# facebookresearch/fast3r

Measured on NVIDIA H100. Metric: views_per_sec, higher is better.
Workload: dtype bf16

## Files before the change

### fast3r_b200/csrc/gemm.cu

```cuda
#include "common.cuh"
#include "f3r_kernels.h"

namespace f3r {

constexpr int BLOCK_M = 128;
constexpr int BLOCK_K = 64;
constexpr int GEMM_THREADS = 384;
constexpr int XCH_STRIDE = 68;

template <int BLOCK_N>
struct GemmCfg {
  static constexpr int kStages = (BLOCK_N == 256) ? 3 : 4;
  static constexpr int kABytes = BLOCK_M * BLOCK_K * 2;
  static constexpr int kBBytes = BLOCK_N * BLOCK_K * 2;
  static constexpr int kStageBytes = kABytes + kBBytes;
  static constexpr int kXchBytes = 64 * XCH_STRIDE * 4;
  static constexpr int kSmemBytes =
      kStages * kStageBytes + 1024  + 1024  + 8 * 4096  + 2 * kXchBytes;
};

struct ResChunk {
  uint4 r0[8];
  uint2 r1[8];
};

__device__ __forceinline__ size_t out_offset(const GemmArgs& p, int m, int col0, int img, int py, int px) {
  if (p.epi == EPI_CONVT) {
    const int ij = col0 / p.ct_cout, o0 = col0 % p.ct_cout, k = p.ct_k;
    const int oy = py * k + ij / k, ox = px * k + ij % k;
    return ((static_cast<size_t>(img) * p.H * k + oy) * (p.W * k) + ox) * p.ct_cout + o0;
  }
  return static_cast<size_t>(m) * p.ldo + col0;
}

__device__ __forceinline__ void prefetch_res(const GemmArgs& p, ResChunk& rc, size_t off_row, bool ok_row, int lane) {
  if (p.res0 == nullptr && p.res1 == nullptr) return;
  const unsigned okmask = __ballot_sync(0xffffffffu, ok_row);
#pragma unroll
  for (int i = 0; i < 8; ++i) {
    const int rr = 4 * i + (lane >> 3);
    const size_t off = __shfl_sync(0xffffffffu, off_row, rr) + (lane & 7) * 4;
    if (!((okmask >> rr) & 1)) continue;
    if (p.res0 != nullptr) {
      if (p.res0_f32) rc.r0[i] = *reinterpret_cast<const uint4*>(static_cast<const float*>(p.res0) + off);
      else {
        const uint2 t = *reinterpret_cast<const uint2*>(static_cast<const __nv_bfloat16*>(p.res0) + off);
        rc.r0[i].x = t.x; rc.r0[i].y = t.y;
      }
    }
    if (p.res1 != nullptr) rc.r1[i] = *reinterpret_cast<const uint2*>(static_cast<const __nv_bfloat16*>(p.res1) + off);
  }
}

__device__ __forceinline__ void gelu_fast(float& x) {
  const float z = __fmul_rn(fabsf(x), 0.70710678118654752440f);
  const float u = fmaf(z, 0.3275911f, 1.0f);
  float t;
  asm("rcp.approx.ftz.f32 %0, %1;" : "=f"(t) : "f"(u));
  float q = fmaf(t, 1.061405429f, -1.453152027f);
  q = fmaf(q, t, 1.421413741f);
  q = fmaf(q, t, -0.284496736f);
  q = fmaf(q, t, 0.254829592f);
  q = __fmul_rn(q, t);
  const float a = __fmul_rn(__fmul_rn(z, z), -1.4426950408889634f);
  float e;
  asm("ex2.approx.ftz.f32 %0, %1;" : "=f"(e) : "f"(a));
  const float r = copysignf(fmaf(q, -e, 1.0f), x);
  const float h = __fmul_rn(x, 0.5f);
  x = fmaf(h, r, h);
}
__device__ __forceinline__ bool epilogue_rows(const GemmArgs& p, float (&v)[32], int m, int col0, bool row_ok,
                                              float (&fin)[4], bool add_bias, const float* w4s) {
  if (p.bias != nullptr && add_bias) {
    const float4* b4 = reinterpret_cast<const float4*>(p.bias + (p.epi == EPI_CONVT ? (col0 % p.ct_cout) : col0));
#pragma unroll
    for (int i = 0; i < 8; ++i) {
      float4 b = __ldg(b4 + i);
      v[4 * i + 0] += b.x; v[4 * i + 1] += b.y; v[4 * i + 2] += b.z; v[4 * i + 3] += b.w;
    }
  }
  if (p.epi == EPI_ROPE && col0 < p.rope_cols && row_ok) {
    const int t = m % p.tok_per_img;
    const int pos = ((col0 >> 5) & 1) ? (t % p.grid_w) : (t / p.grid_w);
    const float4* c4 = reinterpret_cast<const float4*>(p.rope_cos + pos * 16);
    const float4* s4 = reinterpret_cast<const float4*>(p.rope_sin + pos * 16);
#pragma unroll
    for (int i = 0; i < 4; ++i) {
      float4 c = __ldg(c4 + i), s = __ldg(s4 + i);
      float cc[4] = {c.x, c.y, c.z, c.w}, ss[4] = {s.x, s.y, s.z, s.w};
#pragma unroll
      for (int e = 0; e < 4; ++e) {
        const int j = 4 * i + e;
        const float a = v[j], b = v[j + 16];
        v[j] = a * cc[e] - b * ss[e];
        v[j + 16] = b * cc[e] + a * ss[e];
      }
    }
  }
  if (p.epi == EPI_IDXEMB && row_ok) {
    const int id = __ldg(p.emb_ids + (p.tok_per_img > 0 ? m / p.tok_per_img : m));
    const float4* e4 = reinterpret_cast<const float4*>(p.emb_table + static_cast<size_t>(id) * p.N + col0);
#pragma unroll
    for (int i = 0; i < 8; ++i) {
      float4 e = __ldg(e4 + i);
      v[4 * i + 0] += e.x; v[4 * i + 1] += e.y; v[4 * i + 2] += e.z; v[4 * i + 3] += e.w;
    }
  }
  if (p.epi == EPI_FINAL) {
    if (row_ok) {
#pragma unroll
      for (int o = 0; o < 4; ++o) {
        const float4* w = reinterpret_cast<const float4*>(w4s + o * p.N + col0);
        float acc = fin[o];
#pragma unroll
        for (int i = 0; i < 8; ++i) {
          const float4 ww = w[i];
          acc = fmaf(fmaxf(v[4 * i + 0], 0.f), ww.x, acc);
          acc = fmaf(fmaxf(v[4 * i + 1], 0.f), ww.y, acc);
          acc = fmaf(fmaxf(v[4 * i + 2], 0.f), ww.z, acc);
          acc = fmaf(fmaxf(v[4 * i + 3], 0.f), ww.w, acc);
        }
        fin[o] = acc;
      }
    }
    return false;
  }
  return true;
}

__device__ __forceinline__ void epilogue_store(const GemmArgs& p, const float (&v)[32], const ResChunk& rc, uint8_t* stage,
                                               int lane, int m, int col0, size_t off_row, bool ok_row) {
#pragma unroll
  for (int j = 0; j < 8; ++j)
    *reinterpret_cast<float4*>(stage + lane * 128 + ((j ^ (lane & 7)) << 4)) =
        make_float4(v[4 * j], v[4 * j + 1], v[4 * j + 2], v[4 * j + 3]);
  __syncwarp();
  const unsigned okmask = __ballot_sync(0xffffffffu, ok_row);
  const int cj = lane & 7;
  const bool to_b = p.split_col > 0 && col0 >= p.split_col;
#pragma unroll
  for (int i = 0; i < 8; ++i) {
    const int rr = 4 * i + (lane >> 3);
    const size_t off = __shfl_sync(0xffffffffu, off_row, rr) + cj * 4;
    const int mrow = __shfl_sync(0xffffffffu, m, rr);
    if (!((okmask >> rr) & 1)) continue;
    const float4 a = *reinterpret_cast<const float4*>(stage + rr * 128 + ((cj ^ (rr & 7)) << 4));
    float x0 = a.x, x1 = a.y, x2 = a.z, x3 = a.w;
    if (p.res0 != nullptr) {
      if (p.res0_f32) {
        x0 += __uint_as_float(rc.r0[i].x); x1 += __uint_as_float(rc.r0[i].y);
        x2 += __uint_as_float(rc.r0[i].z); x3 += __uint_as_float(rc.r0[i].w);
      } else {
        x0 += bf16_lo(rc.r0[i].x); x1 += bf16_hi(rc.r0[i].x); x2 += bf16_lo(rc.r0[i].y); x3 += bf16_hi(rc.r0[i].y);
      }
    }
    if (p.res1 != nullptr) {
      x0 += bf16_lo(rc.r1[i].x); x1 += bf16_hi(rc.r1[i].x); x2 += bf16_lo(rc.r1[i].y); x3 += bf16_hi(rc.r1[i].y);
    }
    if (p.out1 != nullptr) {
      uint2 o;
      o.x = pack_bf16(fmaxf(x0, 0.f), fmaxf(x1, 0.f));
      o.y = pack_bf16(fmaxf(x2, 0.f), fmaxf(x3, 0.f));
      *reinterpret_cast<uint2*>(static_cast<__nv_bfloat16*>(p.out1) + off) = o;
    }
    if (p.out0 == nullptr) continue;
    if (p.act == ACT_RELU) {
      x0 = fmaxf(x0, 0.f); x1 = fmaxf(x1, 0.f); x2 = fmaxf(x2, 0.f); x3 = fmaxf(x3, 0.f);
    } else if (p.act == ACT_GELU) {
      gelu_fast(x0); gelu_fast(x1); gelu_fast(x2); gelu_fast(x3);
    }
    void* base = p.out0;
    size_t o = off;
    if (to_b) {
      base = p.out0b;
      o = static_cast<size_t>(mrow) * p.ldo_b + (col0 - p.split_col) + cj * 4;
    }
    if (p.out0_f32) {
      *reinterpret_cast<float4*>(static_cast<float*>(base) + o) = make_float4(x0, x1, x2, x3);
    } else {
      uint2 q;
      q.x = pack_bf16(x0, x1);
      q.y = pack_bf16(x2, x3);
      *reinterpret_cast<uint2*>(static_cast<__nv_bfloat16*>(base) + o) = q;
    }
  }
  __syncwarp();
}

__device__ __forceinline__ void epilogue_tma(const GemmArgs& p, float (&v)[32], uint8_t* stage, int lane,
                                             const CUtensorMap* map, bool reduce, int c_col, int c_x, int c_y, int c_img) {
  if (p.act == ACT_RELU) {
#pragma unroll
    for (int i = 0; i < 32; ++i) v[i] = fmaxf(v[i], 0.f);
  } else if (p.act == ACT_GELU) {
#pragma unroll
    for (int i = 0; i < 32; ++i) gelu_fast(v[i]);
  }
  if (lane == 0) tma_store_wait_read();
  __syncwarp();
  if (p.out0_f32) {
#pragma unroll
    for (int j = 0; j < 8; ++j)
      *reinterpret_cast<float4*>(stage + lane * 128 + ((j ^ (lane & 7)) << 4)) =
          make_float4(v[4 * j], v[4 * j + 1], v[4 * j + 2], v[4 * j + 3]);
  } else {
#pragma unroll
    for (int j = 0; j < 4; ++j) {
      uint4 q;
      q.x = pack_bf16(v[8 * j + 0], v[8 * j + 1]);
      q.y = pack_bf16(v[8 * j + 2], v[8 * j + 3]);
      q.z = pack_bf16(v[8 * j + 4], v[8 * j + 5]);
      q.w = pack_bf16(v[8 * j + 6], v[8 * j + 7]);
      *reinterpret_cast<uint4*>(stage + lane * 64 + ((j ^ ((lane >> 1) & 3)) << 4)) = q;
    }
  }
  fence_proxy_async_smem();
  __syncwarp();
  if (lane == 0) {
    if (reduce) tma_reduce_add_4d(map, stage, c_col, c_x, c_y, c_img);
    else tma_store_4d(map, stage, c_col, c_x, c_y, c_img);
    tma_store_commit();
  }
}

template <int BLOCK_N>
__global__ void __launch_bounds__(GEMM_THREADS, 1)
gemm_kernel(const __grid_constant__ CUtensorMap tmap_a, const __grid_constant__ CUtensorMap tmap_b,
            const __grid_constant__ CUtensorMap tmap_o0, const __grid_constant__ CUtensorMap tmap_o0b,
            const __grid_constant__ GemmArgs p) {
  using Cfg = GemmCfg<BLOCK_N>;
  extern __shared__ uint8_t smem_raw[];
  uint8_t* smem = reinterpret_cast<uint8_t*>((reinterpret_cast<uintptr_t>(smem_raw) + 1023) & ~uintptr_t(1023));
  uint8_t* smem_a = smem;
  uint8_t* smem_b = smem + Cfg::kStages * Cfg::kABytes;
  uint64_t* bars = reinterpret_cast<uint64_t*>(smem + Cfg::kStages * Cfg::kStageBytes);
  uint64_t* full_bar = bars;
  uint64_t* empty_bar = bars + Cfg::kStages;
  uint8_t* stage_base = smem + Cfg::kStages * Cfg::kStageBytes + 1024;
  float* fin_smem = reinterpret_cast<float*>(stage_base);
  float* w4_smem = reinterpret_cast<float*>(stage_base + 4096);
  float* xch_base = reinterpret_cast<float*>(stage_base + 8 * 4096);

  const int warp = threadIdx.x >> 5;
  const int lane = threadIdx.x & 31;

  if (threadIdx.x == 0) {
    tma_prefetch_desc(&tmap_a);
    tma_prefetch_desc(&tmap_b);
    for (int s = 0; s < Cfg::kStages; ++s) { mbar_init(&full_bar[s], 1); mbar_init(&empty_bar[s], 2); }
    fence_barrier_init();
  }
  if (p.epi == EPI_FINAL)
    for (int i = threadIdx.x; i < 4 * p.N; i += GEMM_THREADS) w4_smem[i] = __ldg(p.w4 + i);
  __syncthreads();
  pdl_wait();
  pdl_launch_dependents();

  const int num_out_tiles = p.num_m_tiles * p.num_n_tiles;
  const int num_tiles = num_out_tiles * p.k_split;
  const int k_chunks = (p.K + BLOCK_K - 1) / BLOCK_K;
  const int k_iters = p.taps * k_chunks;

  if (warp < 4) {
    asm volatile("setmaxnreg.dec.sync.aligned.u32 40;");
    if (warp == 0 && lane == 0) {
      int stage = 0; uint32_t phase = 0;
      for (int item = blockIdx.x; item < num_tiles; item += gridDim.x) {
        const int tile = item % num_out_tiles, ks = item / num_out_tiles;
        const int it0 = ks * k_iters / p.k_split, it1 = (ks + 1) * k_iters / p.k_split;
        const int mt = tile / p.num_n_tiles, nt = tile % p.num_n_tiles;
        const int tx = mt % p.tiles_x, ty = (mt / p.tiles_x) % p.tiles_y, img = mt / (p.tiles_x * p.tiles_y);
        const int x0 = tx * p.bw, y0 = ty * p.bh, n0 = nt * BLOCK_N;
        for (int it = it0; it < it1; ++it) {
          const int tap = it / k_chunks, kc = it % k_chunks;
          int dy = 0, dx = 0;
          if (p.taps == 9) { dy = tap / 3 - 1; dx = tap % 3 - 1; }
          mbar_wait_relaxed(&empty_bar[stage], phase ^ 1);
          mbar_arrive_expect_tx(&full_bar[stage], Cfg::kStageBytes);
          tma_load_4d(smem_a + stage * Cfg::kABytes, &tmap_a, &full_bar[stage], kc * BLOCK_K, x0 + dx, y0 + dy, img);
          tma_load_3d(smem_b + stage * Cfg::kBBytes, &tmap_b, &full_bar[stage], kc * BLOCK_K, tap, n0);
          if (++stage == Cfg::kStages) { stage = 0; phase ^= 1; }
        }
      }
    }
  } else {
    asm volatile("setmaxnreg.inc.sync.aligned.u32 232;");
    const int cg = (warp - 4) >> 2;
    const int wg_warp = warp & 3;
    const int wg_tid = threadIdx.x & 127;
    const int half = wg_warp >> 1;
    const int r_loc = (wg_warp & 1) * 32 + lane;
    const int r = cg * 64 + r_loc;
    float* xch = xch_base + cg * 64 * XCH_STRIDE;
    uint8_t* stage_buf = stage_base + (warp - 4) * 4096;
    const int bar_id = 1 + cg;
    constexpr int kAcc = BLOCK_N / 2;
    int stage = 0; uint32_t phase = 0;
    for (int item = blockIdx.x; item < num_tiles; item += gridDim.x) {
      const int tile = item % num_out_tiles, ks = item / num_out_tiles;
      const int it0 = ks * k_iters / p.k_split, it1 = (ks + 1) * k_iters / p.k_split;
      const bool add_bias = ks == 0;
      float acc[kAcc];
#pragma unroll
      for (int i = 0; i < kAcc; ++i) acc[i] = 0.f;
      int prev = -1;
      for (int it = it0; it < it1; ++it) {
        mbar_wait(&full_bar[stage], phase);
        const uint64_t a_desc = make_smem_desc_sw128(smem_u32(smem_a + stage * Cfg::kABytes + cg * 64 * 128));
        const uint64_t b_desc = make_smem_desc_sw128(smem_u32(smem_b + stage * Cfg::kBBytes));
        fence_regs(acc);
        wgmma_fence();
#pragma unroll
        for (int k = 0; k < BLOCK_K / 16; ++k) {
          if constexpr (BLOCK_N == 256) wgmma_ss_n256<0>(acc, a_desc + 2 * k, b_desc + 2 * k, 1u);
          else wgmma_ss_n128<0>(acc, a_desc + 2 * k, b_desc + 2 * k, 1u);
        }
        wgmma_commit();
        wgmma_wait<1>();
        fence_regs(acc);
        if (prev >= 0 && wg_tid == 0) mbar_arrive(&empty_bar[prev]);
        prev = stage;
        if (++stage == Cfg::kStages) { stage = 0; phase ^= 1; }
      }
      wgmma_wait<0>();
      fence_regs(acc);
      if (prev >= 0 && wg_tid == 0) mbar_arrive(&empty_bar[prev]);

      const int mt = tile / p.num_n_tiles, nt = tile % p.num_n_tiles;
      const int tx = mt % p.tiles_x, ty = (mt / p.tiles_x) % p.tiles_y, img = mt / (p.tiles_x * p.tiles_y);
      const int px = tx * p.bw + r % p.bw, py = ty * p.bh + r / p.bw;
      const bool row_ok = (px < p.W) && (py < p.H) && (mt < p.num_m_tiles);
      const int m = (img * p.H + py) * p.W + px;
      const int n_valid = min(BLOCK_N / 32, (p.N - nt * BLOCK_N + 31) / 32);
      float fin[4] = {0.f, 0.f, 0.f, 0.f};
#pragma unroll
      for (int cp = 0; cp < BLOCK_N / 64; ++cp) {
        asm volatile("bar.sync %0, 128;" ::"r"(bar_id) : "memory");
        {
          const int fr = wg_warp * 16 + (lane >> 2), fc = 2 * (lane & 3);
#pragma unroll
          for (int j = 0; j < 8; ++j) {
            const int jj = cp * 8 + j;
            *reinterpret_cast<float2*>(xch + fr * XCH_STRIDE + 8 * j + fc) = make_float2(acc[4 * jj], acc[4 * jj + 1]);
            *reinterpret_cast<float2*>(xch + (fr + 8) * XCH_STRIDE + 8 * j + fc) =
                make_float2(acc[4 * jj + 2], acc[4 * jj + 3]);
          }
        }
        asm volatile("bar.sync %0, 128;" ::"r"(bar_id) : "memory");
        const int c = 2 * cp + half;
        if (c >= n_valid) continue;
        const int col0 = nt * BLOCK_N + c * 32;
        float v[32];
#pragma unroll
        for (int i = 0; i < 8; ++i) {
          const float4 t = *reinterpret_cast<const float4*>(xch + r_loc * XCH_STRIDE + half * 32 + 4 * i);
          v[4 * i] = t.x; v[4 * i + 1] = t.y; v[4 * i + 2] = t.z; v[4 * i + 3] = t.w;
        }
        if (epilogue_rows(p, v, m, col0, row_ok, fin, add_bias, w4_smem) && !(p.debug & 1)) {
          if (p.tma_epi) {
            const bool to_b = p.split_col > 0 && col0 >= p.split_col;
            const int r0 = cg * 64 + (wg_warp & 1) * 32;
            epilogue_tma(p, v, stage_buf, lane, to_b ? &tmap_o0b : &tmap_o0, p.tma_epi == 2,
                         to_b ? col0 - p.split_col : col0, tx * p.bw + (r0 & (p.bw - 1)), ty * p.bh + (r0 >> p.bw_log2),
                         mt < p.num_m_tiles ? img : p.NB);
          } else {
            const size_t off = out_offset(p, m, col0, img, py, px);
            ResChunk rc;
            prefetch_res(p, rc, off, row_ok, lane);
            epilogue_store(p, v, rc, stage_buf, lane, m, col0, off, row_ok);
          }
        }
      }
      if (p.epi == EPI_FINAL) {
        float* slot = fin_smem + r * 4;
        if (half == 1) { slot[0] = fin[0]; slot[1] = fin[1]; slot[2] = fin[2]; slot[3] = fin[3]; }
        asm volatile("bar.sync %0, 128;" ::"r"(bar_id) : "memory");
        if (half == 0 && row_ok) {
          const float x = fin[0] + slot[0] + __ldg(p.b4 + 0), y = fin[1] + slot[1] + __ldg(p.b4 + 1);
          const float z = fin[2] + slot[2] + __ldg(p.b4 + 2), c = fin[3] + slot[3] + __ldg(p.b4 + 3);
          const float d = sqrtf(x * x + y * y + z * z);
          const float sc = expm1f(d) / fmaxf(d, 1e-8f);
          float* pt = p.pts + static_cast<size_t>(m) * 3;
          pt[0] = x * sc; pt[1] = y * sc; pt[2] = z * sc;
          p.conf[m] = 1.f + expf(c);
        }
      }
    }
    if (p.tma_epi && lane == 0) tma_store_wait_all();
  }
}

template <int BLOCK_N>
static cudaError_t launch_gemm_t(const CUtensorMap& ta, const CUtensorMap& tb, const CUtensorMap& to0,
                                 const CUtensorMap& to0b, const GemmArgs& a, int num_sms, cudaStream_t stream) {
  const int items = a.num_m_tiles * a.num_n_tiles * a.k_split;
  return launch(gemm_kernel<BLOCK_N>, items < num_sms ? items : num_sms, GEMM_THREADS, GemmCfg<BLOCK_N>::kSmemBytes,
                stream, true, ta, tb, to0, to0b, a);
}

cudaError_t launch_gemm(int block_n, const CUtensorMap& ta, const CUtensorMap& tb, const CUtensorMap& to0,
                        const CUtensorMap& to0b, const GemmArgs& a, int num_sms, cudaStream_t stream) {
  if (block_n == 256) return launch_gemm_t<256>(ta, tb, to0, to0b, a, num_sms, stream);
  return launch_gemm_t<128>(ta, tb, to0, to0b, a, num_sms, stream);
}

}
```

Baseline: 149.1.

## Run GEMM epilogue directly on MMA fragments instead of shared-memory transpose

The epilogue now applies bias, RoPE and index embeddings directly on the wgmma accumulator fragment layout. This removes the per-chunk shared-memory exchange and the two 128-thread barriers that converted fragments to row-per-thread form. Warps are paired to share a double-buffered TMA staging area synchronized with 64-thread named barriers. Freeing the exchange buffer lets BLOCK_N=256 use four pipeline stages instead of three, while the FINAL epilogue keeps the old exchange path for BLOCK_N=128. In exchange the indexing and synchronization become more complex.

```diff
diff --git a/fast3r_b200/csrc/gemm.cu b/fast3r_b200/csrc/gemm.cu
--- a/fast3r_b200/csrc/gemm.cu
+++ b/fast3r_b200/csrc/gemm.cu
@@ -10,18 +10,19 @@
 
 template <int BLOCK_N>
 struct GemmCfg {
-  static constexpr int kStages = (BLOCK_N == 256) ? 3 : 4;
+  static constexpr int kStages = 4;
   static constexpr int kABytes = BLOCK_M * BLOCK_K * 2;
   static constexpr int kBBytes = BLOCK_N * BLOCK_K * 2;
   static constexpr int kStageBytes = kABytes + kBBytes;
-  static constexpr int kXchBytes = 64 * XCH_STRIDE * 4;
+  static constexpr int kXchBytes = (BLOCK_N == 128) ? 2 * 64 * XCH_STRIDE * 4 : 0;
   static constexpr int kSmemBytes =
-      kStages * kStageBytes + 1024  + 1024  + 8 * 4096  + 2 * kXchBytes;
+      kStages * kStageBytes + 1024  + 1024  + 8 * 4096  + kXchBytes;
 };
+static_assert(GemmCfg<256>::kSmemBytes <= 227 * 1024 && GemmCfg<128>::kSmemBytes <= 227 * 1024, "shared memory per CTA");
 
 struct ResChunk {
-  uint4 r0[8];
-  uint2 r1[8];
+  uint4 r0[4];
+  uint2 r1[4];
 };
 
 __device__ __forceinline__ size_t out_offset(const GemmArgs& p, int m, int col0, int img, int py, int px) {
@@ -33,14 +34,21 @@
   return static_cast<size_t>(m) * p.ldo + col0;
 }
 
-__device__ __forceinline__ void prefetch_res(const GemmArgs& p, ResChunk& rc, size_t off_row, bool ok_row, int lane) {
+struct FragRows {
+  int m[2];
+  int px[2], py[2];
+  bool ok[2];
+};
+
+__device__ __forceinline__ void prefetch_res(const GemmArgs& p, ResChunk& rc, const size_t (&off_row)[2], const FragRows& rows,
+                                             int lane) {
   if (p.res0 == nullptr && p.res1 == nullptr) return;
-  const unsigned okmask = __ballot_sync(0xffffffffu, ok_row);
-#pragma unroll
-  for (int i = 0; i < 8; ++i) {
-    const int rr = 4 * i + (lane >> 3);
-    const size_t off = __shfl_sync(0xffffffffu, off_row, rr) + (lane & 7) * 4;
-    if (!((okmask >> rr) & 1)) continue;
+  const unsigned okmask[2] = {__ballot_sync(0xffffffffu, rows.ok[0]), __ballot_sync(0xffffffffu, rows.ok[1])};
+#pragma unroll
+  for (int i = 0; i < 4; ++i) {
+    const int src = 4 * ((4 * i + (lane >> 3)) & 7);
+    const size_t off = __shfl_sync(0xffffffffu, off_row[i >> 1], src) + (lane & 7) * 4;
+    if (!((okmask[i >> 1] >> src) & 1)) continue;
     if (p.res0 != nullptr) {
       if (p.res0_f32) rc.r0[i] = *reinterpret_cast<const uint4*>(static_cast<const float*>(p.res0) + off);
       else {
@@ -69,81 +77,111 @@
   const float h = __fmul_rn(x, 0.5f);
   x = fmaf(h, r, h);
 }
-__device__ __forceinline__ bool epilogue_rows(const GemmArgs& p, float (&v)[32], int m, int col0, bool row_ok,
-                                              float (&fin)[4], bool add_bias, const float* w4s) {
+template <int kAcc>
+__device__ __forceinline__ void epilogue_frag(const GemmArgs& p, float (&acc)[kAcc], int c, int col0, const FragRows& rows,
+                                              int lane, bool add_bias) {
+  const int t2 = 2 * (lane & 3);
   if (p.bias != nullptr && add_bias) {
-    const float4* b4 = reinterpret_cast<const float4*>(p.bias + (p.epi == EPI_CONVT ? (col0 % p.ct_cout) : col0));
+    const float2* b2 = reinterpret_cast<const float2*>(p.bias + (p.epi == EPI_CONVT ? (col0 % p.ct_cout) : col0) + t2);
+#pragma unroll
+    for (int jl = 0; jl < 4; ++jl) {
+      const float2 b = __ldg(b2 + 4 * jl);
+#pragma unroll
+      for (int h = 0; h < 2; ++h) { acc[16 * c + 4 * jl + 2 * h] += b.x; acc[16 * c + 4 * jl + 2 * h + 1] += b.y; }
+    }
+  }
+  if (p.epi == EPI_ROPE && col0 < p.rope_cols) {
+#pragma unroll
+    for (int h = 0; h < 2; ++h) {
+      if (!rows.ok[h]) continue;
+      const int t = rows.m[h] % p.tok_per_img;
+      const int pos = ((col0 >> 5) & 1) ? (t % p.grid_w) : (t / p.grid_w);
+      const float2* c2 = reinterpret_cast<const float2*>(p.rope_cos + pos * 16 + t2);
+      const float2* s2 = reinterpret_cast<const float2*>(p.rope_sin + pos * 16 + t2);
+#pragma unroll
+      for (int jl = 0; jl < 2; ++jl) {
+        const float2 cs = __ldg(c2 + 4 * jl), sn = __ldg(s2 + 4 * jl);
+#pragma unroll
+        for (int e = 0; e < 2; ++e) {
+          float& x = acc[16 * c + 4 * jl + 2 * h + e];
+          float& y = acc[16 * c + 4 * (jl + 2) + 2 * h + e];
+          const float a = x, b = y, cc = e ? cs.y : cs.x, ss = e ? sn.y : sn.x;
+          x = fmaf(a, cc, -__fmul_rn(b, ss));
+          y = fmaf(a, ss, __fmul_rn(b, cc));
+        }
+      }
+    }
+  }
+  if (p.epi == EPI_IDXEMB) {
+#pragma unroll
+    for (int h = 0; h < 2; ++h) {
+      if (!rows.ok[h]) continue;
+      const int m = rows.m[h];
+      const int id = __ldg(p.emb_ids + (p.tok_per_img > 0 ? m / p.tok_per_img : m));
+      const float2* e2 = reinterpret_cast<const float2*>(p.emb_table + static_cast<size_t>(id) * p.N + col0 + t2);
+#pragma unroll
+      for (int jl = 0; jl < 4; ++jl) {
+        const float2 e = __ldg(e2 + 4 * jl);
+        acc[16 * c + 4 * jl + 2 * h] += e.x; acc[16 * c + 4 * jl + 2 * h + 1] += e.y;
+      }
+    }
+  }
+}
+
+__device__ __forceinline__ void final_rows(const GemmArgs& p, float (&v)[32], int col0, bool row_ok, float (&fin)[4],
+                                           const float* w4s) {
+  if (p.bias != nullptr) {
+    const float4* b4 = reinterpret_cast<const float4*>(p.bias + col0);
 #pragma unroll
     for (int i = 0; i < 8; ++i) {
       float4 b = __ldg(b4 + i);
       v[4 * i + 0] += b.x; v[4 * i + 1] += b.y; v[4 * i + 2] += b.z; v[4 * i + 3] += b.w;
     }
   }
-  if (p.epi == EPI_ROPE && col0 < p.rope_cols && row_ok) {
-    const int t = m % p.tok_per_img;
-    const int pos = ((col0 >> 5) & 1) ? (t % p.grid_w) : (t / p.grid_w);
-    const float4* c4 = reinterpret_cast<const float4*>(p.rope_cos + pos * 16);
-    const float4* s4 = reinterpret_cast<const float4*>(p.rope_sin + pos * 16);
-#pragma unroll
-    for (int i = 0; i < 4; ++i) {
-      float4 c = __ldg(c4 + i), s = __ldg(s4 + i);
-      float cc[4] = {c.x, c.y, c.z, c.w}, ss[4] = {s.x, s.y, s.z, s.w};
-#pragma unroll
-      for (int e = 0; e < 4; ++e) {
-        const int j = 4 * i + e;
-        const float a = v[j], b = v[j + 16];
-        v[j] = a * cc[e] - b * ss[e];
-        v[j + 16] = b * cc[e] + a * ss[e];
-      }
-    }
-  }
-  if (p.epi == EPI_IDXEMB && row_ok) {
-    const int id = __ldg(p.emb_ids + (p.tok_per_img > 0 ? m / p.tok_per_img : m));
-    const float4* e4 = reinterpret_cast<const float4*>(p.emb_table + static_cast<size_t>(id) * p.N + col0);
+  if (!row_ok) return;
+#pragma unroll
+  for (int o = 0; o < 4; ++o) {
+    const float4* w = reinterpret_cast<const float4*>(w4s + o * p.N + col0);
+    float acc = fin[o];
 #pragma unroll
     for (int i = 0; i < 8; ++i) {
-      float4 e = __ldg(e4 + i);
-      v[4 * i + 0] += e.x; v[4 * i + 1] += e.y; v[4 * i + 2] += e.z; v[4 * i + 3] += e.w;
-    }
-  }
-  if (p.epi == EPI_FINAL) {
-    if (row_ok) {
-#pragma unroll
-      for (int o = 0; o < 4; ++o) {
-        const float4* w = reinterpret_cast<const float4*>(w4s + o * p.N + col0);
-        float acc = fin[o];
-#pragma unroll
-        for (int i = 0; i < 8; ++i) {
-          const float4 ww = w[i];
-          acc = fmaf(fmaxf(v[4 * i + 0], 0.f), ww.x, acc);
-          acc = fmaf(fmaxf(v[4 * i + 1], 0.f), ww.y, acc);
-          acc = fmaf(fmaxf(v[4 * i + 2], 0.f), ww.z, acc);
-          acc = fmaf(fmaxf(v[4 * i + 3], 0.f), ww.w, acc);
-        }
-        fin[o] = acc;
-      }
-    }
-    return false;
-  }
-  return true;
-}
-
-__device__ __forceinline__ void epilogue_store(const GemmArgs& p, const float (&v)[32], const ResChunk& rc, uint8_t* stage,
-                                               int lane, int m, int col0, size_t off_row, bool ok_row) {
-#pragma unroll
-  for (int j = 0; j < 8; ++j)
-    *reinterpret_cast<float4*>(stage + lane * 128 + ((j ^ (lane & 7)) << 4)) =
-        make_float4(v[4 * j], v[4 * j + 1], v[4 * j + 2], v[4 * j + 3]);
+      const float4 ww = w[i];
+      acc = fmaf(fmaxf(v[4 * i + 0], 0.f), ww.x, acc);
+      acc = fmaf(fmaxf(v[4 * i + 1], 0.f), ww.y, acc);
+      acc = fmaf(fmaxf(v[4 * i + 2], 0.f), ww.z, acc);
+      acc = fmaf(fmaxf(v[4 * i + 3], 0.f), ww.w, acc);
+    }
+    fin[o] = acc;
+  }
+}
+
+template <int kAcc>
+__device__ __forceinline__ void stage_frag_f32(const float (&acc)[kAcc], int c, uint8_t* stage, int row0, int lane) {
+  const int q = lane >> 2, t = lane & 3;
+#pragma unroll
+  for (int jl = 0; jl < 4; ++jl)
+#pragma unroll
+    for (int h = 0; h < 2; ++h)
+      *reinterpret_cast<float2*>(stage + (row0 + 8 * h) * 128 + (((2 * jl + (t >> 1)) ^ q) << 4) + (t & 1) * 8) =
+          make_float2(acc[16 * c + 4 * jl + 2 * h], acc[16 * c + 4 * jl + 2 * h + 1]);
+}
+
+template <int kAcc>
+__device__ __forceinline__ void epilogue_store(const GemmArgs& p, const float (&acc)[kAcc], int c, const ResChunk& rc,
+                                               uint8_t* stage, int lane, const FragRows& rows, int col0,
+                                               const size_t (&off_row)[2]) {
+  stage_frag_f32(acc, c, stage, lane >> 2, lane);
   __syncwarp();
-  const unsigned okmask = __ballot_sync(0xffffffffu, ok_row);
+  const unsigned okmask[2] = {__ballot_sync(0xffffffffu, rows.ok[0]), __ballot_sync(0xffffffffu, rows.ok[1])};
   const int cj = lane & 7;
   const bool to_b = p.split_col > 0 && col0 >= p.split_col;
 #pragma unroll
-  for (int i = 0; i < 8; ++i) {
+  for (int i = 0; i < 4; ++i) {
     const int rr = 4 * i + (lane >> 3);
-    const size_t off = __shfl_sync(0xffffffffu, off_row, rr) + cj * 4;
-    const int mrow = __shfl_sync(0xffffffffu, m, rr);
-    if (!((okmask >> rr) & 1)) continue;
+    const int src = 4 * (rr & 7);
+    const size_t off = __shfl_sync(0xffffffffu, off_row[i >> 1], src) + cj * 4;
+    const int mrow = __shfl_sync(0xffffffffu, rows.m[i >> 1], src);
+    if (!((okmask[i >> 1] >> src) & 1)) continue;
     const float4 a = *reinterpret_cast<const float4*>(stage + rr * 128 + ((cj ^ (rr & 7)) << 4));
     float x0 = a.x, x1 = a.y, x2 = a.z, x3 = a.w;
     if (p.res0 != nullptr) {
@@ -187,39 +225,83 @@
   __syncwarp();
 }
 
-__device__ __forceinline__ void epilogue_tma(const GemmArgs& p, float (&v)[32], uint8_t* stage, int lane,
-                                             const CUtensorMap* map, bool reduce, int c_col, int c_x, int c_y, int c_img) {
+template <int kAcc>
+__device__ __forceinline__ void epilogue_tma(const GemmArgs& p, float (&acc)[kAcc], int c, uint8_t* stage, int row0, int lane,
+                                             bool leader, int pair_bar, const CUtensorMap* map, bool reduce, int c_col,
+                                             int c_x, int c_y, int c_img) {
   if (p.act == ACT_RELU) {
 #pragma unroll
-    for (int i = 0; i < 32; ++i) v[i] = fmaxf(v[i], 0.f);
+    for (int i = 0; i < 16; ++i) acc[16 * c + i] = fmaxf(acc[16 * c + i], 0.f);
   } else if (p.act == ACT_GELU) {
 #pragma unroll
-    for (int i = 0; i < 32; ++i) gelu_fast(v[i]);
-  }
-  if (lane == 0) tma_store_wait_read();
-  __syncwarp();
+    for (int i = 0; i < 16; ++i) gelu_fast(acc[16 * c + i]);
+  }
   if (p.out0_f32) {
-#pragma unroll
-    for (int j = 0; j < 8; ++j)
-      *reinterpret_cast<float4*>(stage + lane * 128 + ((j ^ (lane & 7)) << 4)) =
-          make_float4(v[4 * j], v[4 * j + 1], v[4 * j + 2], v[4 * j + 3]);
+    stage_frag_f32(acc, c, stage, row0, lane);
   } else {
-#pragma unroll
-    for (int j = 0; j < 4; ++j) {
-      uint4 q;
-      q.x = pack_bf16(v[8 * j + 0], v[8 * j + 1]);
-      q.y = pack_bf16(v[8 * j + 2], v[8 * j + 3]);
-      q.z = pack_bf16(v[8 * j + 4], v[8 * j + 5]);
-      q.w = pack_bf16(v[8 * j + 6], v[8 * j + 7]);
-      *reinterpret_cast<uint4*>(stage + lane * 64 + ((j ^ ((lane >> 1) & 3)) << 4)) = q;
-    }
+    const int q = lane >> 2, t = lane & 3;
+#pragma unroll
+    for (int jl = 0; jl < 4; ++jl)
+#pragma unroll
+      for (int h = 0; h < 2; ++h)
+        *reinterpret_cast<uint32_t*>(stage + (row0 + 8 * h) * 64 + ((jl ^ ((q >> 1) & 3)) << 4) + 4 * t) =
+            pack_bf16(acc[16 * c + 4 * jl + 2 * h], acc[16 * c + 4 * jl + 2 * h + 1]);
   }
   fence_proxy_async_smem();
-  __syncwarp();
-  if (lane == 0) {
+  if (leader) tma_store_wait_read();
+  asm volatile("bar.sync %0, 64;" ::"r"(pair_bar) : "memory");
+  if (leader) {
     if (reduce) tma_reduce_add_4d(map, stage, c_col, c_x, c_y, c_img);
     else tma_store_4d(map, stage, c_col, c_x, c_y, c_img);
     tma_store_commit();
+  }
+}
+
+__device__ __forceinline__ void final_epilogue(const GemmArgs& p, const float (&acc)[64], int cg, int wg_warp, int lane,
+                                               float* xch, float* fin_smem, const float* w4s, int n_valid, int nt, int tx,
+                                               int ty, int img, int mt) {
+  const int half = wg_warp >> 1;
+  const int r_loc = (wg_warp & 1) * 32 + lane;
+  const int r = cg * 64 + r_loc;
+  const int bar_id = 1 + cg;
+  const int px = tx * p.bw + r % p.bw, py = ty * p.bh + r / p.bw;
+  const bool row_ok = (px < p.W) && (py < p.H) && (mt < p.num_m_tiles);
+  const int m = (img * p.H + py) * p.W + px;
+  float fin[4] = {0.f, 0.f, 0.f, 0.f};
+#pragma unroll
+  for (int cp = 0; cp < 2; ++cp) {
+    asm volatile("bar.sync %0, 128;" ::"r"(bar_id) : "memory");
+    {
+      const int fr = wg_warp * 16 + (lane >> 2), fc = 2 * (lane & 3);
+#pragma unroll
+      for (int j = 0; j < 8; ++j) {
+        const int jj = cp * 8 + j;
+        *reinterpret_cast<float2*>(xch + fr * XCH_STRIDE + 8 * j + fc) = make_float2(acc[4 * jj], acc[4 * jj + 1]);
+        *reinterpret_cast<float2*>(xch + (fr + 8) * XCH_STRIDE + 8 * j + fc) = make_float2(acc[4 * jj + 2], acc[4 * jj + 3]);
+      }
+    }
+    asm volatile("bar.sync %0, 128;" ::"r"(bar_id) : "memory");
+    const int c = 2 * cp + half;
+    if (c >= n_valid) continue;
+    float v[32];
+#pragma unroll
+    for (int i = 0; i < 8; ++i) {
+      const float4 t = *reinterpret_cast<const float4*>(xch + r_loc * XCH_STRIDE + half * 32 + 4 * i);
+      v[4 * i] = t.x; v[4 * i + 1] = t.y; v[4 * i + 2] = t.z; v[4 * i + 3] = t.w;
+    }
+    final_rows(p, v, nt * 128 + c * 32, row_ok, fin, w4s);
+  }
+  float* slot = fin_smem + r * 4;
+  if (half == 1) { slot[0] = fin[0]; slot[1] = fin[1]; slot[2] = fin[2]; slot[3] = fin[3]; }
+  asm volatile("bar.sync %0, 128;" ::"r"(bar_id) : "memory");
+  if (half == 0 && row_ok) {
+    const float x = fin[0] + slot[0] + __ldg(p.b4 + 0), y = fin[1] + slot[1] + __ldg(p.b4 + 1);
+    const float z = fin[2] + slot[2] + __ldg(p.b4 + 2), c = fin[3] + slot[3] + __ldg(p.b4 + 3);
+    const float d = sqrtf(x * x + y * y + z * z);
+    const float sc = expm1f(d) / fmaxf(d, 1e-8f);
+    float* pt = p.pts + static_cast<size_t>(m) * 3;
+    pt[0] = x * sc; pt[1] = y * sc; pt[2] = z * sc;
+    p.conf[m] = 1.f + expf(c);
   }
 }
 
@@ -288,12 +370,12 @@
     const int cg = (warp - 4) >> 2;
     const int wg_warp = warp & 3;
     const int wg_tid = threadIdx.x & 127;
-    const int half = wg_warp >> 1;
-    const int r_loc = (wg_warp & 1) * 32 + lane;
-    const int r = cg * 64 + r_loc;
-    float* xch = xch_base + cg * 64 * XCH_STRIDE;
-    uint8_t* stage_buf = stage_base + (warp - 4) * 4096;
-    const int bar_id = 1 + cg;
+    const int pair = (warp - 4) >> 1;
+    const int frag_r0 = cg * 64 + wg_warp * 16 + (lane >> 2);
+    uint8_t* stage_pair = stage_base + pair * 8192;
+    const bool pair_leader = (wg_warp & 1) == 0 && lane == 0;
+    const int pair_bar = 3 + pair;
+    int sbuf = 0;
     constexpr int kAcc = BLOCK_N / 2;
     int stage = 0; uint32_t phase = 0;
     for (int item = blockIdx.x; item < num_tiles; item += gridDim.x) {
@@ -328,65 +410,63 @@
 
       const int mt = tile / p.num_n_tiles, nt = tile % p.num_n_tiles;
       const int tx = mt % p.tiles_x, ty = (mt / p.tiles_x) % p.tiles_y, img = mt / (p.tiles_x * p.tiles_y);
-      const int px = tx * p.bw + r % p.bw, py = ty * p.bh + r / p.bw;
-      const bool row_ok = (px < p.W) && (py < p.H) && (mt < p.num_m_tiles);
-      const int m = (img * p.H + py) * p.W + px;
       const int n_valid = min(BLOCK_N / 32, (p.N - nt * BLOCK_N + 31) / 32);
-      float fin[4] = {0.f, 0.f, 0.f, 0.f};
+      if constexpr (BLOCK_N == 128) {
+        if (p.epi == EPI_FINAL) {
+          final_epilogue(p, acc, cg, wg_warp, lane, xch_base + cg * 64 * XCH_STRIDE, fin_smem, w4_smem, n_valid, nt, tx, ty,
+                         img, mt);
+          continue;
+        }
+      }
+      FragRows rows;
+#pragma unroll
+      for (int h = 0; h < 2; ++h) {
+        const int r = frag_r0 + 8 * h;
+        rows.px[h] = tx * p.bw + (r & (p.bw - 1));
+        rows.py[h] = ty * p.bh + (r >> p.bw_log2);
+        rows.ok[h] = (rows.px[h] < p.W) && (rows.py[h] < p.H) && (mt < p.num_m_tiles);
+        rows.m[h] = (img * p.H + rows.py[h]) * p.W + rows.px[h];
+      }
 #pragma unroll
       for (int cp = 0; cp < BLOCK_N / 64; ++cp) {
-        asm volatile("bar.sync %0, 128;" ::"r"(bar_id) : "memory");
-        {
-          const int fr = wg_warp * 16 + (lane >> 2), fc = 2 * (lane & 3);
-#pragma unroll
-          for (int j = 0; j < 8; ++j) {
-            const int jj = cp * 8 + j;
-            *reinterpret_cast<float2*>(xch + fr * XCH_STRIDE + 8 * j + fc) = make_float2(acc[4 * jj], acc[4 * jj + 1]);
-            *reinterpret_cast<float2*>(xch + (fr + 8) * XCH_STRIDE + 8 * j + fc) =
-                make_float2(acc[4 * jj + 2], acc[4 * jj + 3]);
+        const int nc = min(2, n_valid - 2 * cp);
+        if (nc <= 0) continue;
+#pragma unroll
+        for (int e = 0; e < 2; ++e)
+          if (e < nc) epilogue_frag(p, acc, 2 * cp + e, nt * BLOCK_N + (2 * cp + e) * 32, rows, lane, add_bias);
+        if (p.debug & 1) continue;
+        if (p.tma_epi) {
+#pragma unroll
+          for (int e = 0; e < 2; ++e) {
+            if (e >= nc) continue;
+            const int col0 = nt * BLOCK_N + (2 * cp + e) * 32;
+            const bool to_b = p.split_col > 0 && col0 >= p.split_col;
+            const int r0 = cg * 64 + (wg_warp >> 1) * 32;
+            epilogue_tma(p, acc, 2 * cp + e, stage_pair + sbuf * 4096, (wg_warp & 1) * 16 + (lane >> 2), lane, pair_leader,
+                         pair_bar, to_b ? &tmap_o0b : &tmap_o0, p.tma_epi == 2, to_b ? col0 - p.split_col : col0,
+                         tx * p.bw + (r0 & (p.bw - 1)), ty * p.bh + (r0 >> p.bw_log2), mt < p.num_m_tiles ? img : p.NB);
+            sbuf ^= 1;
           }
+        } else {
+          size_t off[2][2];
+          ResChunk rc[2];
+#pragma unroll
+          for (int e = 0; e < 2; ++e) {
+            if (e >= nc) continue;
+            const int col0 = nt * BLOCK_N + (2 * cp + e) * 32;
+#pragma unroll
+            for (int h = 0; h < 2; ++h) off[e][h] = out_offset(p, rows.m[h], col0, img, rows.py[h], rows.px[h]);
+            prefetch_res(p, rc[e], off[e], rows, lane);
+          }
+#pragma unroll
+          for (int e = 0; e < 2; ++e)
+            if (e < nc)
+              epilogue_store(p, acc, 2 * cp + e, rc[e], stage_pair + e * 4096 + (wg_warp & 1) * 2048, lane, rows,
+                             nt * BLOCK_N + (2 * cp + e) * 32, off[e]);
         }
-        asm volatile("bar.sync %0, 128;" ::"r"(bar_id) : "memory");
-        const int c = 2 * cp + half;
-        if (c >= n_valid) continue;
-        const int col0 = nt * BLOCK_N + c * 32;
-        float v[32];
-#pragma unroll
-        for (int i = 0; i < 8; ++i) {
-          const float4 t = *reinterpret_cast<const float4*>(xch + r_loc * XCH_STRIDE + half * 32 + 4 * i);
-          v[4 * i] = t.x; v[4 * i + 1] = t.y; v[4 * i + 2] = t.z; v[4 * i + 3] = t.w;
-        }
-        if (epilogue_rows(p, v, m, col0, row_ok, fin, add_bias, w4_smem) && !(p.debug & 1)) {
-          if (p.tma_epi) {
-            const bool to_b = p.split_col > 0 && col0 >= p.split_col;
-            const int r0 = cg * 64 + (wg_warp & 1) * 32;
-            epilogue_tma(p, v, stage_buf, lane, to_b ? &tmap_o0b : &tmap_o0, p.tma_epi == 2,
-                         to_b ? col0 - p.split_col : col0, tx * p.bw + (r0 & (p.bw - 1)), ty * p.bh + (r0 >> p.bw_log2),
-                         mt < p.num_m_tiles ? img : p.NB);
-          } else {
-            const size_t off = out_offset(p, m, col0, img, py, px);
-            ResChunk rc;
-            prefetch_res(p, rc, off, row_ok, lane);
-            epilogue_store(p, v, rc, stage_buf, lane, m, col0, off, row_ok);
-          }
-        }
-      }
-      if (p.epi == EPI_FINAL) {
-        float* slot = fin_smem + r * 4;
-        if (half == 1) { slot[0] = fin[0]; slot[1] = fin[1]; slot[2] = fin[2]; slot[3] = fin[3]; }
-        asm volatile("bar.sync %0, 128;" ::"r"(bar_id) : "memory");
-        if (half == 0 && row_ok) {
-          const float x = fin[0] + slot[0] + __ldg(p.b4 + 0), y = fin[1] + slot[1] + __ldg(p.b4 + 1);
-          const float z = fin[2] + slot[2] + __ldg(p.b4 + 2), c = fin[3] + slot[3] + __ldg(p.b4 + 3);
-          const float d = sqrtf(x * x + y * y + z * z);
-          const float sc = expm1f(d) / fmaxf(d, 1e-8f);
-          float* pt = p.pts + static_cast<size_t>(m) * 3;
-          pt[0] = x * sc; pt[1] = y * sc; pt[2] = z * sc;
-          p.conf[m] = 1.f + expf(c);
-        }
-      }
-    }
-    if (p.tma_epi && lane == 0) tma_store_wait_all();
+      }
+    }
+    if (p.tma_epi && pair_leader) tma_store_wait_all();
   }
 }
 
```

Result: faster. 151.5 (median of 6 runs) (+1.6%).
